# hccho2/Tacotron-Wavenet-Vocoder-Korean

Hardware: AMD Instinct MI355X
Metric: WaveNet autoregressive audio samples/sec at 24 kHz, batch=8 (higher is better)
Workload: dtype f32

## Files before the change

tacotron-wavenet-vocoder-korean_amd/csrc/twv_dpp.hpp:

```cpp
#pragma once
#include <hip/hip_runtime.h>
#include "twv_math.hpp"

#define TWV_ALIGN8 "\t.p2align 3\n"

namespace twv {

__host__ __device__ inline int dpp_a(int n) { return 4 * (n >> 1) + (n & 1); }
__host__ __device__ inline int dpp_conv_out(int lane) { const int r = lane >> 4, n = lane & 15; return ((r >> 1) ? 32 : 0) + dpp_a(n) + ((r & 1) ? 2 : 0); }
__host__ __device__ inline int dpp_dense_out(int lane) { return (lane & 15) + 16 * (lane >> 5); }
__host__ __device__ inline int dpp_dense_k(int lane, int i) { return dpp_a(i) + (((lane >> 4) & 1) ? 2 : 0); }
__host__ __device__ inline int dpp_z_index(int lane) { return dpp_a(lane & 15) + (((lane >> 4) & 1) ? 2 : 0); }

__device__ __forceinline__ float dot32_dpp(const float (&w)[32], float xa, float xb, float init = 0.0f)
{
    float c0 = init, c1 = 0.0f, c2 = 0.0f, c3 = 0.0f;
    asm volatile(
        "s_nop 1\n" TWV_ALIGN8
        "v_fmac_f32_dpp %0, %4, %5 row_newbcast:0 row_mask:0xf bank_mask:0xf\n"
        "v_fmac_f32_dpp %1, %4, %6 row_newbcast:1 row_mask:0xf bank_mask:0xf\n"
        "v_fmac_f32_dpp %2, %4, %7 row_newbcast:2 row_mask:0xf bank_mask:0xf\n"
        "v_fmac_f32_dpp %3, %4, %8 row_newbcast:3 row_mask:0xf bank_mask:0xf\n"
        "v_fmac_f32_dpp %0, %4, %9 row_newbcast:4 row_mask:0xf bank_mask:0xf\n"
        "v_fmac_f32_dpp %1, %4, %10 row_newbcast:5 row_mask:0xf bank_mask:0xf\n"
// ... 153 lines not shown
    TWV_FMAC12_DPP(c, d, e, xb0, xb1, xb2, wa, wb, wc, 24, 8, 9, 10, 11);
    TWV_FMAC12_DPP(c, d, e, xb0, xb1, xb2, wa, wb, wc, 28, 12, 13, 14, 15);
    ra = (c[0] + c[1]) + (c[2] + c[3]);
    rb = (d[0] + d[1]) + (d[2] + d[3]);
    rc = (e[0] + e[1]) + (e[2] + e[3]);
}

__device__ __forceinline__ float dot16_dpp(const float (&w)[16], float z, float init = 0.0f)
{
    float c0 = init, c1 = 0.0f;
    asm volatile(
        "s_nop 1\n" TWV_ALIGN8
        "v_fmac_f32_dpp %0, %2, %3 row_newbcast:0 row_mask:0xf bank_mask:0xf\n"
        "v_fmac_f32_dpp %1, %2, %4 row_newbcast:1 row_mask:0xf bank_mask:0xf\n"
        "v_fmac_f32_dpp %0, %2, %5 row_newbcast:2 row_mask:0xf bank_mask:0xf\n"
        "v_fmac_f32_dpp %1, %2, %6 row_newbcast:3 row_mask:0xf bank_mask:0xf\n"
        "v_fmac_f32_dpp %0, %2, %7 row_newbcast:4 row_mask:0xf bank_mask:0xf\n"
        "v_fmac_f32_dpp %1, %2, %8 row_newbcast:5 row_mask:0xf bank_mask:0xf\n"
        "v_fmac_f32_dpp %0, %2, %9 row_newbcast:6 row_mask:0xf bank_mask:0xf\n"
        "v_fmac_f32_dpp %1, %2, %10 row_newbcast:7 row_mask:0xf bank_mask:0xf\n"
        "v_fmac_f32_dpp %0, %2, %11 row_newbcast:8 row_mask:0xf bank_mask:0xf\n"
        "v_fmac_f32_dpp %1, %2, %12 row_newbcast:9 row_mask:0xf bank_mask:0xf\n"
        "v_fmac_f32_dpp %0, %2, %13 row_newbcast:10 row_mask:0xf bank_mask:0xf\n"
        "v_fmac_f32_dpp %1, %2, %14 row_newbcast:11 row_mask:0xf bank_mask:0xf\n"
        "v_fmac_f32_dpp %0, %2, %15 row_newbcast:12 row_mask:0xf bank_mask:0xf\n"
        "v_fmac_f32_dpp %1, %2, %16 row_newbcast:13 row_mask:0xf bank_mask:0xf\n"
        "v_fmac_f32_dpp %0, %2, %17 row_newbcast:14 row_mask:0xf bank_mask:0xf\n"
        "v_fmac_f32_dpp %1, %2, %18 row_newbcast:15 row_mask:0xf bank_mask:0xf"
        : "+v"(c0), "+v"(c1)
        : "v"(z), "v"(w[0]), "v"(w[1]), "v"(w[2]), "v"(w[3]), "v"(w[4]), "v"(w[5]), "v"(w[6]), "v"(w[7]), "v"(w[8]), "v"(w[9]), "v"(w[10]), "v"(w[11]), "v"(w[12]), "v"(w[13]), "v"(w[14]), "v"(w[15]));
    return c0 + c1;
}

__device__ __forceinline__ float dot32_dpp_chain(const float (&w)[32], float xa, float xb, float init)
{
    float c0 = init, c1, c2, c3;
    asm volatile(
        "s_nop 1\n" TWV_ALIGN8
        "v_fmac_f32_dpp %0, %4, %5 row_newbcast:0 row_mask:0xf bank_mask:0xf\n"
        "v_mul_f32_dpp %1, %4, %6 row_newbcast:1 row_mask:0xf bank_mask:0xf\n"
        "v_mul_f32_dpp %2, %4, %7 row_newbcast:2 row_mask:0xf bank_mask:0xf\n"
        "v_mul_f32_dpp %3, %4, %8 row_newbcast:3 row_mask:0xf bank_mask:0xf\n"
        "v_fmac_f32_dpp %0, %4, %9 row_newbcast:4 row_mask:0xf bank_mask:0xf\n"
        "v_fmac_f32_dpp %1, %4, %10 row_newbcast:5 row_mask:0xf bank_mask:0xf\n"
        "v_fmac_f32_dpp %2, %4, %11 row_newbcast:6 row_mask:0xf bank_mask:0xf\n"
        "v_fmac_f32_dpp %3, %4, %12 row_newbcast:7 row_mask:0xf bank_mask:0xf\n"
        "v_fmac_f32_dpp %0, %4, %13 row_newbcast:8 row_mask:0xf bank_mask:0xf\n"
        "v_fmac_f32_dpp %1, %4, %14 row_newbcast:9 row_mask:0xf bank_mask:0xf\n"
        "v_fmac_f32_dpp %2, %4, %15 row_newbcast:10 row_mask:0xf bank_mask:0xf\n"
        "v_fmac_f32_dpp %3, %4, %16 row_newbcast:11 row_mask:0xf bank_mask:0xf\n"
        "v_fmac_f32_dpp %0, %4, %17 row_newbcast:12 row_mask:0xf bank_mask:0xf\n"
        "v_fmac_f32_dpp %1, %4, %18 row_newbcast:13 row_mask:0xf bank_mask:0xf\n"
        "v_fmac_f32_dpp %2, %4, %19 row_newbcast:14 row_mask:0xf bank_mask:0xf\n"
        "v_fmac_f32_dpp %3, %4, %20 row_newbcast:15 row_mask:0xf bank_mask:0xf"
        : "+v"(c0), "=&v"(c1), "=&v"(c2), "=&v"(c3)
        : "v"(xa), "v"(w[0]), "v"(w[1]), "v"(w[2]), "v"(w[3]), "v"(w[4]), "v"(w[5]), "v"(w[6]), "v"(w[7]), "v"(w[8]), "v"(w[9]), "v"(w[10]), "v"(w[11]), "v"(w[12]), "v"(w[13]), "v"(w[14]), "v"(w[15]));
    asm volatile(
        TWV_ALIGN8
        "v_fmac_f32_dpp %0, %4, %5 row_newbcast:0 row_mask:0xf bank_mask:0xf\n"
        "v_fmac_f32_dpp %1, %4, %6 row_newbcast:1 row_mask:0xf bank_mask:0xf\n"
        "v_fmac_f32_dpp %2, %4, %7 row_newbcast:2 row_mask:0xf bank_mask:0xf\n"
        "v_fmac_f32_dpp %3, %4, %8 row_newbcast:3 row_mask:0xf bank_mask:0xf\n"
        "v_fmac_f32_dpp %0, %4, %9 row_newbcast:4 row_mask:0xf bank_mask:0xf\n"
        "v_fmac_f32_dpp %1, %4, %10 row_newbcast:5 row_mask:0xf bank_mask:0xf\n"
        "v_fmac_f32_dpp %2, %4, %11 row_newbcast:6 row_mask:0xf bank_mask:0xf\n"
        "v_fmac_f32_dpp %3, %4, %12 row_newbcast:7 row_mask:0xf bank_mask:0xf\n"
// ... 111 lines not shown
```

tacotron-wavenet-vocoder-korean_amd/csrc/twv_wavenet_xcd.hip:

```cpp
#include <hip/hip_runtime.h>
#include <stdint.h>
#include <string>
#include <type_traits>
#include "../../include/twv_amd.h"
#include "twv_layout.hpp"
#include "twv_math.hpp"
#include "twv_dev.hpp"
#include "twv_dpp.hpp"
#include "twv_categorical.hpp"
#include "twv_xcd.hpp"

using namespace twv;

#ifndef TWV_CHAIN_PAD
#define TWV_CHAIN_PAD 0
#endif
#ifndef TWV_WATCHDOG_LOG2
#define TWV_WATCHDOG_LOG2 21
#endif
#define TWV_STR2(x) #x
#define TWV_STR(x) TWV_STR2(x)
namespace {

typedef __attribute__((address_space(1))) unsigned long long gu64;
// ... 107 lines not shown
        "v_fmac_f32_dpp %1, %4, %6 row_newbcast:1 row_mask:0xf bank_mask:0xf\n"
        "v_fmac_f32_dpp %2, %4, %7 row_newbcast:2 row_mask:0xf bank_mask:0xf\n"
        "v_fmac_f32_dpp %3, %4, %8 row_newbcast:3 row_mask:0xf bank_mask:0xf\n"
        "v_fmac_f32_dpp %0, %4, %9 row_newbcast:4 row_mask:0xf bank_mask:0xf\n"
        "v_fmac_f32_dpp %1, %4, %10 row_newbcast:5 row_mask:0xf bank_mask:0xf\n"
        "v_fmac_f32_dpp %2, %4, %11 row_newbcast:6 row_mask:0xf bank_mask:0xf\n"
        "v_fmac_f32_dpp %3, %4, %12 row_newbcast:7 row_mask:0xf bank_mask:0xf\n"
        "v_fmac_f32_dpp %0, %4, %13 row_newbcast:8 row_mask:0xf bank_mask:0xf\n"
        "v_fmac_f32_dpp %1, %4, %14 row_newbcast:9 row_mask:0xf bank_mask:0xf\n"
        "v_fmac_f32_dpp %2, %4, %15 row_newbcast:10 row_mask:0xf bank_mask:0xf\n"
        "v_fmac_f32_dpp %3, %4, %16 row_newbcast:11 row_mask:0xf bank_mask:0xf\n"
        "v_fmac_f32_dpp %0, %4, %17 row_newbcast:12 row_mask:0xf bank_mask:0xf\n"
        "v_fmac_f32_dpp %1, %4, %18 row_newbcast:13 row_mask:0xf bank_mask:0xf\n"
        "v_fmac_f32_dpp %2, %4, %19 row_newbcast:14 row_mask:0xf bank_mask:0xf\n"
        "v_fmac_f32_dpp %3, %4, %20 row_newbcast:15 row_mask:0xf bank_mask:0xf"
        : "+v"(c0), "+v"(c1), "+v"(c2), "+v"(c3)
        : "v"(xb), "v"(w[0]), "v"(w[1]), "v"(w[2]), "v"(w[3]), "v"(w[4]), "v"(w[5]), "v"(w[6]), "v"(w[7]), "v"(w[8]), "v"(w[9]), "v"(w[10]), "v"(w[11]), "v"(w[12]), "v"(w[13]), "v"(w[14]), "v"(w[15]));
    return (c0 + c1) + (c2 + c3);
}

#define XSTAMP(cond_, slot_) do { if ((INSTR & 1) && a.prof != nullptr && b == a.prof_stream && t < a.prof_steps && lane == 0 && (cond_)) a.prof[(long long)t * 64 + (slot_)] = wall_clock64(); } while (0)

#define WACC_DECL() unsigned long long wacc_[6] = {0, 0, 0, 0, 0, 0}, w0_ = 0, wt0_ = 0; if (INSTR & 4) wt0_ = __builtin_amdgcn_s_memtime()
#define WACC_T0() do { if (INSTR & 4) w0_ = __builtin_amdgcn_s_memtime(); } while (0)
#define WACC_T1(i_) do { if (INSTR & 4) wacc_[i_] += __builtin_amdgcn_s_memtime() - w0_; } while (0)
constexpr int kTraceStep = 2000;
#define WTRACE(cond_, slot_) do { if ((INSTR & 4) && a.prof != nullptr && t == kTraceStep && (cond_) && lane == 0) a.prof[2048 + (slot_)] = wall_clock64(); } while (0)
#define WACC_OUT(prof_, slot_, wave_) do { if ((INSTR & 4) && (prof_) != nullptr && (slot_) >= 0 && lane == 0) {                 \
        unsigned long long* o_ = (prof_) + (((slot_) * 8 + (wave_)) * 8);                                                        \
        o_[0] = __builtin_amdgcn_s_memtime() - wt0_;                                                                             \
        o_[1] = wacc_[0]; o_[2] = wacc_[1]; o_[3] = wacc_[2]; o_[4] = wacc_[3]; o_[5] = wacc_[4]; o_[6] = wacc_[5]; } } while (0)
#define XMARK(role_, stage_) do { if ((INSTR & 1) && lane == 0) xb_store(rs, (int)XcdExch::MARK + (role_) * 8 + (int)(threadIdx.x >> 6), 0, (unsigned)t + 1u, (float)(stage_)); } while (0)

enum { ROLE_CHAIN = 0, ROLE_SERVICE = 1, ROLE_SKIP0 = 2, ROLE_CONV0 = 10, ROLE_LC0 = 18 };
constexpr int kXcdStreamsPerXcd = kXcdStreams / 8;

struct XArgs {
    XcdLaunch p;
    int n_lc_wg, lc_lpw;
    int total_roles;
};

template <int NS> struct XStreams { rsrc_t rs[NS]; int b[NS]; };
__device__ __forceinline__ rsrc_t exch_rsrc(const XcdLaunch& a, int b)
{
    return __builtin_amdgcn_make_buffer_rsrc(a.exch + (long long)b * XcdExch::WORDS, 0, (int)(XcdExch::WORDS * 8), 0x00020000);
}
struct XLazyRs { const XcdLaunch* a; int xcc, ns; __device__ __forceinline__ rsrc_t operator[](int k) const { return exch_rsrc(*a, xcc + 8 * (k < ns ? k : 0)); } };
struct XLazyB { int xcc, ns; __device__ __forceinline__ int operator[](int k) const { return xcc + 8 * (k < ns ? k : 0); } };
template <int NS> struct XStreamsLazy { XLazyRs rs; XLazyB b; };
constexpr int kSkipLdsWords = 32 * 64;
constexpr int kConvLdsFloats = 16 * 64 + 64;

constexpr int kChainLpw = 5;
template <int INSTR, bool ALL, bool FORCED, bool SEG1, bool TWOSEG, int NC, bool ONEHOT = false, bool HEAD = false, bool CONT = false>
__device__ __forceinline__ void chain_role(const XArgs& xa, int b, rsrc_t rs)
{
    const XcdLaunch& a = xa.p;
    const Layout& L = a.lay;
    const int w = __builtin_amdgcn_readfirstlane(threadIdx.x >> 6), lane = threadIdx.x & 63;
    const int NL = L.NL, T = a.T;
    const bool use_bias = L.use_bias != 0, has_gc = L.G > 0, has_lc = L.L > 0;
    constexpr bool forced = FORCED;
    constexpr int kLayerWaves = kXcdSeg0Layers / kChainLpw;
    const int l0 = (SEG1 ? kXcdSeg0Layers : 0) + kChainLpw * w;
    const int lw0 = kChainLpw * w;
    const int cap = (HEAD || w >= kLayerWaves) ? 0 : kChainLpw;
    int nl = NL - l0;
    nl = nl < 0 ? 0 : (nl > cap ? cap : nl);
    const int nlc = NC >= 0 ? NC : nl;
    const bool next_has = (l0 + nl < NL);
    constexpr bool head = HEAD;
// ... 677 lines not shown
            if (!havez) qz = xb_load_t<BAR>(rs, (int)XcdExch::ZX + last_layer * 128, zc_lane * 2);
            q = xb_load_t<BAR>(rs, (int)XcdExch::H1 + v * 64, lane);
            if (!havez && __all(g_tag(qz) == tag)) {
                const auto sw = __builtin_amdgcn_permlane32_swap((unsigned)qz, (unsigned)qz, false, false);
                val = dot32_dpp(wl, __uint_as_float(sw[0]), __uint_as_float(sw[1]));
                if (use_bias) val = val + bl;
                havez = true;
                saw_z = true;
            }
            if (havez && __all(g_tag(q) == tag)) break;
            if (!poll_tick<BAR>(pl, 61)) break;
            if (!havez) __builtin_amdgcn_s_sleep(1);
        }
        const float tot = g_val(q) + val;
        const float h = tot > 0.0f ? tot : 0.0f;
        q = (unsigned long long)__float_as_uint(h);
    } else {
        for (;;) {
            q = xb_load_t<BAR>(rs, (int)XcdExch::H1 + v * 64, lane);
            if (__all(g_tag(q) == tag)) break;
            if (!poll_tick<BAR>(pl, 61)) break;
            __builtin_amdgcn_s_sleep(1);
        }
    }
    return q;
}
__device__ __forceinline__ void conv1_load_last_skip(const XcdLaunch& a, const int v, const int lane, Tile& wl, float& bl)
{
    const Layout& L = a.lay;
    const long long lb = L.off_layer0 + (long long)(L.NL - 1) * L.layer_stride;
    load_tile(wl, a.P + lb + LayerOff::SK + (long long)v * kTile, lane);
    if (L.use_bias != 0) bl = a.P[lb + LayerOff::SK + (long long)L.NSJ * kTile + v * 64 + lane];
}

template <int INSTR, int NS, bool BAR = false, class SX = XStreams<NS>, int KF = 0>
__device__ __forceinline__ void conv1_role(const XArgs& xa, const SX& sx, int g, const int ns_rt = NS, const int prof_slot = -1)
{
    const XcdLaunch& a = xa.p;
    const Layout& L = a.lay;
    const int v = __builtin_amdgcn_readfirstlane(threadIdx.x >> 6), lane = threadIdx.x & 63;
    const int T = a.T, NCH = L.NCH;
    const bool use_bias = L.use_bias != 0;
    Poll pl{sx.rs[0], a.status, 0, false};
    constexpr int O_PART = 0, O_CNT = 16 * 64;
    if (threadIdx.x < NS) LDSI(threadIdx.x * kConvLdsFloats + O_CNT) = 0;
    __syncthreads();
    const int c0 = 2 * v, c1 = 2 * v + 1;
    Tile ta, tb;
    load_tile(ta, a.P + L.off_w1 + ((long long)g * NCH + c0) * kTile, lane);
    load_tile(tb, a.P + L.off_w1 + ((long long)g * NCH + c1) * kTile, lane);
    const bool summer = v < 2;
    float b1v = 0.0f;
    Tile t2;
    if (summer) {
        if (use_bias) b1v = a.P[L.off_b1 + g * 64 + lane];
        load_tile(t2, a.P + L.off_w2 + (long long)(2 * g + v) * kTile, lane);
    }
    Tile wl;
    float bl = 0.0f;
    if (KF > 0) conv1_load_last_skip(a, v, lane, wl, bl);
    const int zc_lane = lane_of_z((lane < 32 ? 0 : 16) + (lane & 15));
    unsigned long long t_arr = 0, period = 0;
    WACC_DECL();
    for (int t = 0; t < T && !pl.dead; ++t) {
        asm volatile(".p2align 6");
        const unsigned tag = (unsigned)t + 1u;
        WACC_T0();
        if (period) nap_until(t_arr + period - (period >> 3));
        WACC_T1(0);
#pragma unroll
        for (int k = 0; k < NS; ++k) {
            if (pl.dead) break;
            if (k >= ns_rt) break;
            const rsrc_t rs = sx.rs[k];
            const int b = sx.b[k];
            const int ob = k * kConvLdsFloats;
            pl.rs = rs;
            XMARK(ROLE_CONV0 + g, 1);
            WACC_T0();
            bool saw_z = false;
            const unsigned long long q = conv1_fetch_h1<KF, BAR>(pl, rs, v, lane, tag, L.NL - 1, zc_lane, wl.w, bl, use_bias, saw_z);
            (void)saw_z;
            WACC_T1(1);
            WTRACE(prof_slot >= 0 && k == 0, 400 + g * 8 + v);
            unsigned long long now_arr = 0;
            if (k == 0) now_arr = __builtin_amdgcn_s_memtime();
            XSTAMP(g == 0 && v == 0, 22);
            const unsigned hq = (unsigned)q;
            const auto p16 = __builtin_amdgcn_permlane16_swap(hq, hq, false, false);
            const auto pa = __builtin_amdgcn_permlane32_swap(p16[0], p16[0], false, false);
            const auto pb = __builtin_amdgcn_permlane32_swap(p16[1], p16[1], false, false);
            float r0, r1;
            dot32_dpp_x2(ta.w, __uint_as_float(pa[0]), __uint_as_float(pb[0]), tb.w, __uint_as_float(pa[1]), __uint_as_float(pb[1]), r0, r1);
            lds[ob + O_PART + c0 * 64 + lane] = r0;
            lds[ob + O_PART + c1 * 64 + lane] = r1;
            asm volatile("" ::: "memory");
            if (lane == 0) __hip_atomic_fetch_add(&LDSI(ob + O_CNT), 1, __ATOMIC_RELAXED, __HIP_MEMORY_SCOPE_WORKGROUP);
            if (k == 0) {
                const unsigned long long d = now_arr - t_arr;
                period = (t_arr != 0 && d < (1ull << 18)) ? d : 0;
                t_arr = now_arr;
            }
            XSTAMP(g == 0 && v == 0, 23);
            XMARK(ROLE_CONV0 + g, 2);
            if (summer) {
                WACC_T0();
                pl.it = 0;
                while (LDSVI(ob + O_CNT) < 8 * (t + 1)) { if (!poll_tick<BAR>(pl, 62)) break; }
                WACC_T1(2);
                asm volatile("" ::: "memory");
                XSTAMP(g == 0 && v == 0, 24);
                float cp[16];
#pragma unroll
                for (int ch = 0; ch < 16; ++ch) cp[ch] = lds[ob + O_PART + ch * 64 + lane];
                __builtin_amdgcn_sched_barrier(0);
                float r = cp[0];
#pragma unroll
                for (int ch = 1; ch < 16; ++ch) r = r + cp[ch];
                if (use_bias) r = r + b1v;
                const float h = r > 0.0f ? r : 0.0f;
                const float p = (v == 0) ? dot_readlane_pipe(t2, h) : dot_readlane_pipe32(t2, h);
                if (lane < 32) xb_store(rs, (int)XcdExch::PT, (g * 32 + lane) * 2 + v, tag, p);
                WTRACE(prof_slot >= 0 && k == 0, 480 + g * 2 + v);
                XSTAMP(g == 0 && v == 0, 25);
            }
        }
    }
    if (pl.dead && lane == 0) {
#pragma unroll
        for (int k = 0; k < NS; ++k) xb_store(sx.rs[k], (int)XcdExch::CTRL + 1, 0, 1u, 0.0f);
    }
    WACC_OUT(a.prof, prof_slot, v);
}

constexpr int kConvQLdsFloats = 16 * 64 + 64 + 8 * 64;
template <int INSTR, int NS, int KF = 0>
__device__ __forceinline__ void conv1_onehot_role(const XArgs& xa, const XStreams<NS>& sx, int g)
{
    const XcdLaunch& a = xa.p;
    const Layout& L = a.lay;
    const int v = __builtin_amdgcn_readfirstlane(threadIdx.x >> 6), lane = threadIdx.x & 63;
    const int T = a.T, NCH = L.NCH;
    const bool use_bias = L.use_bias != 0;
    Poll pl{sx.rs[0], a.status, 0, false};
    constexpr int O_PART = 0, O_CNT = 16 * 64, O_P2 = 16 * 64 + 64;
    if (threadIdx.x < NS) { LDSI(threadIdx.x * kConvQLdsFloats + O_CNT) = 0; LDSI(threadIdx.x * kConvQLdsFloats + O_CNT + 1) = 0; }
    __syncthreads();
    const int c0 = 2 * v, c1 = 2 * v + 1;
    Tile ta, tb;
    load_tile(ta, a.P + L.off_w1 + ((long long)g * NCH + c0) * kTile, lane);
    load_tile(tb, a.P + L.off_w1 + ((long long)g * NCH + c1) * kTile, lane);
    float w2[32];
    {
        const int ch2 = lane < 32 ? c0 : c1;
        const f32x4* src = reinterpret_cast<const f32x4*>(a.P + L.off_w2 + ((long long)(g >> 1) * NCH + ch2) * kTile) + ((g & 1) * 32 + (lane & 31));
#pragma unroll
        for (int q = 0; q < 8; ++q) { const f32x4 w = src[q * 64]; w2[4 * q] = w.x; w2[4 * q + 1] = w.y; w2[4 * q + 2] = w.z; w2[4 * q + 3] = w.w; }
    }
    float b1v = 0.0f, b2v = 0.0f;
    if (use_bias && v == 0) b1v = a.P[L.off_b1 + g * 64 + lane];
    if (use_bias && v == 1 && lane < 32) b2v = a.P[L.off_b2 + g * 32 + lane];
    Tile wl;
    float bl = 0.0f;
    if (KF > 0) conv1_load_last_skip(a, v, lane, wl, bl);
    const int zc_lane = lane_of_z((lane < 32 ? 0 : 16) + (lane & 15));
// ... 120 lines not shown
        }
    }
    const int o_row = v * 256;
    const int n16 = lane & 15;
    int ph[4] = {0, 0, 0, 0}, frame = 0;
    const int n_up = L.n_up;
    int hop = 1;
    for (int i = 0; i < n_up; ++i) hop *= L.up[i];
    const long long need_rows = (mode == XLC_MEL) ? ((long long)T + hop - 1) / hop : T;
    if (rows < need_rows) {
        if (lane == 0) {
            atomicMax(a.status, 71);
#pragma unroll
            for (int k = 0; k < NS; ++k) xb_store(sx.rs[k], (int)XcdExch::CTRL + 1, 0, 1u, 0.0f);
        }
        return;
    }
    WACC_DECL();
    for (int u = 0; u < T && !pl.dead; ++u) {
        const int t = u;
        float k0[4] = {0.f, 0.f, 0.f, 0.f}, k1[4] = {0.f, 0.f, 0.f, 0.f};
        if (mode != XLC_UPSAMPLED) {
#pragma unroll
            for (int i = 0; i < 4; ++i)
                if (i < n_up) { k0[i] = a.P[L.off_up[i] + ph[i] * 2 + 0]; k1[i] = a.P[L.off_up[i] + ph[i] * 2 + 1]; }
        }
        WACC_T0();
        if (u + 3 - kXcdLcRing > 0) {
#pragma unroll
            for (int k = 0; k < NS; ++k) {
                if (k >= ns_rt) break;
                const rsrc_t rs = sx.rs[k];
                pl.rs = rs;
                XMARK(ROLE_LC0 + wg, 1);
                pl.it = 0;
                while (!pl.dead) {
                    const unsigned long long q = xb_load_t<BAR>(rs, (int)XcdExch::CTRL, 0);
                    if ((int)g_tag(q) >= u + 3 - kXcdLcRing) break;
                    if (!poll_tick<BAR>(pl, 72)) break;
                    __builtin_amdgcn_s_sleep(16);
                }
            }
            if (pl.dead) break;
        }
        WACC_T1(0);
        float rowa[NS], rowb[NS];
#pragma unroll
        for (int k = 0; k < NS; ++k) {
            rowa[k] = 0.0f; rowb[k] = 0.0f;
            if (k >= ns_rt) continue;
            const float* src = payload + ((long long)sx.b[k] * rows + (mode == XLC_UPSAMPLED ? u : frame)) * Lc;
            rowa[k] = lane < Lc ? src[lane] : 0.0f;
            rowb[k] = 64 + lane < Lc ? src[64 + lane] : 0.0f;
        }
#pragma unroll
        for (int k = 0; k < NS; ++k) {
            if (k >= ns_rt) break;
            const rsrc_t rs = sx.rs[k];
            const int b = sx.b[k];
            int o_cur = o_row;
            lds[o_cur + lane] = rowa[k];
            lds[o_cur + 64 + lane] = rowb[k];
            if (mode != XLC_UPSAMPLED) {
#pragma unroll
                for (int i = 0; i < 4; ++i) {
                    if (i < n_up) {
                        const int o_nxt = (o_cur == o_row) ? o_row + 128 : o_row;
// ... 84 lines not shown
            f = atomicAdd(decision, 0);
            if (f != 0) break;
            __builtin_amdgcn_s_sleep(32);
        }
        if (f == 0) {
            const int old = atomicCAS(decision, 0, 2);
            f = old == 0 ? 2 : old;
            if (old == 0) atomicMax(a.status, 90);
        }
        s_go = (f == 1) ? 1 : 0;
    }
    __syncthreads();
    return s_go != 0;
}

template <int INSTR, bool BIGK, bool ONE, bool ONEHOT = false>
__global__ void __launch_bounds__(512) wn_xcd_generate_kernel(XArgs xa)
{
    const XcdLaunch& a = xa.p;
    unsigned xcc;
    asm volatile("s_getreg_b32 %0, hwreg(HW_REG_XCC_ID)" : "=s"(xcc));
    xcc &= 15u;
    int ticket = 0;
    if (threadIdx.x == 0) ticket = (xcc < (unsigned)a.B && xcc < 8u) ? atomicAdd(a.roles + xcc, 1) : 1 << 20;
    ticket = __shfl(ticket, 0);
    __shared__ int s_ticket;
    if (threadIdx.x == 0) s_ticket = ticket;
    for (int i = threadIdx.x; i < kXcdStreamsPerXcd * kSkipLdsWords * 2 + 64; i += blockDim.x) lds[i] = 0.0f;
    __syncthreads();
    ticket = s_ticket;
    const int ns = xcc < (unsigned)a.B && xcc < 8u ? (a.B - (int)xcc + 7) / 8 : 0;
    constexpr int nseg = BIGK ? 2 : 1;
    const int nchain = ns * nseg;
    if (ticket >= nchain + ns + 16 + xa.n_lc_wg) return;
    if (!roles_resident(xa)) return;
    const bool forced = a.forced != nullptr;
    auto exch_of = [&](int b) { return __builtin_amdgcn_make_buffer_rsrc(a.exch + (long long)b * XcdExch::WORDS, 0, (int)(XcdExch::WORDS * 8), 0x00020000); };
    if (ticket < nchain + ns) {
        const int k = ticket < nchain ? ticket / nseg : ticket - nchain;
        const int b = (int)xcc + 8 * k;
        const rsrc_t rs = exch_of(b);
        if (ticket < nchain) {
            if (ticket % nseg == 0) {
                const int wv = __builtin_amdgcn_readfirstlane(threadIdx.x >> 6);
                const int nlw = a.lay.NL - kChainLpw * wv;
                if (wv == 7) {
                    if (forced) chain_role<INSTR, true, true, false, BIGK, 0, ONEHOT, true>(xa, b, rs);
                    else chain_role<INSTR, true, false, false, BIGK, 0, ONEHOT, true>(xa, b, rs);
                }
                else if (wv >= kXcdSeg0Layers / kChainLpw || nlw <= 0) {}
                else if (forced) chain_role<INSTR, true, true, false, BIGK, -1, ONEHOT>(xa, b, rs);
                else if (nlw > kChainLpw) chain_role<INSTR, true, false, false, BIGK, kChainLpw, ONEHOT, false, true>(xa, b, rs);
                else if (nlw == kChainLpw) chain_role<INSTR, true, false, false, BIGK, kChainLpw, ONEHOT, false, false>(xa, b, rs);
                else chain_role<INSTR, true, false, false, BIGK, -1, ONEHOT>(xa, b, rs);
            } else if constexpr (BIGK) {
                const int wv = __builtin_amdgcn_readfirstlane(threadIdx.x >> 6);
                if (forced) chain_role<INSTR, true, true, true, true, -1>(xa, b, rs);
                else if (a.lay.NL - kXcdSeg0Layers - kChainLpw * wv >= kChainLpw) chain_role<INSTR, true, false, true, true, kChainLpw>(xa, b, rs);
                else chain_role<INSTR, true, false, true, true, -1>(xa, b, rs);
            }
        }
        else service_role<INSTR, BIGK>(xa, b, rs);
        return;
    }
    const int role = ticket - nchain - ns;
    auto shared_roles = [&](auto nsc) {
        constexpr int NS = decltype(nsc)::value;
        XStreams<NS> sx;
#pragma unroll
        for (int k = 0; k < NS; ++k) { sx.b[k] = (int)xcc + 8 * k; sx.rs[k] = exch_of(sx.b[k]); }
        constexpr int KF = TWV_XCD_KF;
        constexpr bool kUnfolded = KF == 0 || INSTR == 0;
        const bool fold = KF > 0 && (a.lay.NL > KF || !kUnfolded);
        if (role < 8) {
            if (!forced) {
                if (fold) skip_role<INSTR, NS, BIGK, KF>(xa, sx, role);
                else if constexpr (kUnfolded) skip_role<INSTR, NS, BIGK, 0>(xa, sx, role);
            }
        }
        else if (role < 16) {
            if (!forced) {
                if constexpr (ONEHOT) {
                    if (fold) conv1_onehot_role<INSTR, NS, KF>(xa, sx, role - 8);
                    else if constexpr (kUnfolded) conv1_onehot_role<INSTR, NS, 0>(xa, sx, role - 8);
                }
                else if (fold) conv1_role<INSTR, NS, false, XStreams<NS>, KF>(xa, sx, role - 8);
                else if constexpr (kUnfolded) conv1_role<INSTR, NS>(xa, sx, role - 8);
            }
        }
        else lc_role<INSTR, NS, BIGK>(xa, sx, role - 16);
    };
    if constexpr (BIGK) {
        if (ns == 1) shared_roles(std::integral_constant<int, 1>{});
        else shared_roles(std::integral_constant<int, 2>{});
    } else if constexpr (ONE) {
        shared_roles(std::integral_constant<int, 1>{});
    } else {
        if (ns == 1) shared_roles(std::integral_constant<int, 1>{});
        else if (ns == 2) shared_roles(std::integral_constant<int, 2>{});
        else if (ns == 3) shared_roles(std::integral_constant<int, 3>{});
        else shared_roles(std::integral_constant<int, 4>{});
    }
}

#define MMARK(rs_, slot_, stage_) do { if ((INSTR & 2) && lane == 0) xb_store(rs_, (int)XcdExch::MARK + (slot_), 0, (unsigned)t + 1u, (float)(stage_)); } while (0)
constexpr int kMS = 2;
constexpr int kManyChains = 6;
constexpr int kManyPerXcd = kMS * kManyChains;
constexpr int kM_BOX = 10;
constexpr int kM_OWD = 4096;
constexpr int kM_OGC = kM_OWD + kXcdSeg0Layers * 1024;
constexpr int kM_OHS = kM_OGC + kMS * kXcdSeg0Layers * 64;
constexpr int kManyChainLds = kM_OHS + kMS * 9 * 64;
constexpr int kManySkipData4 = kManyPerXcd * 8 * 64;
constexpr int kManySkipLds = kManySkipData4 * 4 + kManyPerXcd * 8 * 64;
constexpr int kManyLds = kManyChainLds > kManySkipLds ? kManyChainLds : kManySkipLds;


template <int INSTR>
__device__ __forceinline__ float many_sample(const XcdLaunch& a, const Layout& L, Poll& pl, rsrc_t rs, int lane, unsigned tag, float b2v,
                                             float s_lnl, float s_tq, bool use_bias, int b, int NL)
{
    const int half = lane >> 5;
// ... 825 lines not shown
                if (c == 0) v = blob[lb + (oc < 32 ? L.c_bf : L.c_bg) + (oc & 31)];
                else if (c == 1) v = blob[lb + L.c_bd + od];
            }
            dst[L.off_xl + i] = v;
        } else {
            const int e = (int)(i - per_layer * L.NL);
            const int q = e >> 8, lane = (e >> 2) & 63, c = e & 3;
            const int k = 4 * q + c;
            if (k < L.ifw) v = blob[L.c_causal + k * 32 + dpp_dense_out(lane)];
            dst[L.off_xc + e] = v;
        }
    }
}

}

namespace twv {

bool xcd_model_ok(const Layout& L)
{
    const bool head_ok = L.scalar ? (L.ifw == 32 && L.O <= 32 && L.NOJ == 1) : (L.Q == 256 && L.O == 256);
    return head_ok && L.S == 512 && L.NL >= 1 && L.NL <= kXcdMaxLayers && L.NLC <= 4;
}
static bool xcd_many_lc_fits(const Layout& L) { return (long long)kManyPerXcd * (L.n_up + 1) * L.NLC * 32 <= kManyLds / 8; }
int xcd_max_streams(const Layout& L) { return L.NL > kXcdSeg0Layers ? kXcdStreams / 2 : (L.scalar && xcd_many_lc_fits(L) ? kXcdManyStreams : kXcdStreams); }
static int lc_layers_per_wave(const Layout& L) { const int n = L.NLC > 0 ? (L.NL > kXcdSeg0Layers ? 6 : 4) / L.NLC : 1; return n < 1 ? 1 : (n > 4 ? 4 : n); }
int xcd_lc_workgroups(const Layout& L)
{
    if (L.L == 0) return 0;
    const int lpw = lc_layers_per_wave(L);
    const int waves = (L.NL + lpw - 1) / lpw;
    return (waves + 7) / 8;
}
int xcd_workgroups_per_stream(const Layout& L) { return ROLE_LC0 + xcd_lc_workgroups(L); }
size_t xcd_exchange_bytes(int batch) { return (size_t)batch * XcdExch::WORDS * 8 + 64; }
void xcd_pack(float* packed, const float* blob, const Layout& L, hipStream_t st)
{
    hipLaunchKernelGGL(wn_xcd_pack_kernel, dim3(512), dim3(256), 0, st, packed, blob, L);
}
bool xcd_uses_many(const Layout& L, int batch, int many_opt)
{
    return L.scalar && (batch > kXcdStreams || many_opt == 1 || (many_opt == 0 && batch >= kXcdManyFrom)) && L.NL <= kXcdSeg0Layers && xcd_many_lc_fits(L);
}
int xcd_launch(const XcdLaunch& p, hipStream_t st)
{
    XArgs xa;
    xa.p = p;
    xa.n_lc_wg = xcd_lc_workgroups(p.lay);
    xa.lc_lpw = lc_layers_per_wave(p.lay);
    const bool many = xcd_uses_many(p.lay, p.B, p.many);
    xa.total_roles = 0;
    for (int x = 0; x < 8 && x < p.B; ++x) {
        const int ns = (p.B - x + 7) / 8;
        if (many) xa.total_roles += 2 * ((ns + kMS - 1) / kMS) + 16 + xa.n_lc_wg;
        else xa.total_roles += ns * (p.lay.NL > kXcdSeg0Layers ? 2 : 1) + ns + 16 + xa.n_lc_wg;
    }
    const size_t shm = many ? (size_t)kManyLds * 4 : p.lay.NL > kXcdSeg0Layers ? (size_t)159 * 1024 : (size_t)kXcdChainLdsFloats * 4;
    int dev = 0, cus = 256;
    hipDeviceProp_t prop;
    if (hipGetDevice(&dev) == hipSuccess && hipGetDeviceProperties(&prop, dev) == hipSuccess) cus = prop.multiProcessorCount;
    else (void)hipGetLastError();
    const int grid = 2 * cus;
    const int instr = (p.prof != nullptr ? 1 : 0) | (p.dbg != nullptr ? 2 : 0);
    auto go = [&](auto kern) {
        (void)hipFuncSetAttribute((const void*)kern, hipFuncAttributeMaxDynamicSharedMemorySize, (int)shm);
        (void)hipGetLastError();
        hipLaunchKernelGGL(kern, dim3(grid), dim3(512), shm, st, xa);
    };
    if (!many && instr != 0 && p.lay.NL <= TWV_XCD_KF)
        return twv_fail(TWV_E_UNSUPPORTED, "layer dumps / phase stamps of the XCD kernel need a model of at least two layers (set option \"xcd\" = 0 for the generic kernel)");
    if (many) {
        if (p.B > kXcdManyStreams) return twv_fail(TWV_E_UNSUPPORTED, "the many-streams XCD kernel takes at most 96 streams");
        if (instr == 3) return twv_fail(TWV_E_UNSUPPORTED, "layer dumps and wait accounting are separate builds of the many-streams kernel");
        if (instr == 1) go(wn_xcd_many_kernel<4>);
        else if (instr == 2) go(wn_xcd_many_kernel<2>);
        else go(wn_xcd_many_kernel<0>);
    }
    else if (!p.lay.scalar) {
        if (p.B > (p.lay.NL > kXcdSeg0Layers ? kXcdStreams / 2 : kXcdStreams)) return twv_fail(TWV_E_UNSUPPORTED, "the one-hot XCD kernel takes at most 32 streams (16 above 30 layers)");
        if (instr == 3 || (instr != 0 && p.lay.NL > kXcdSeg0Layers))
            return twv_fail(TWV_E_UNSUPPORTED, "the one-hot XCD kernel has layer dumps OR phase stamps, up to 30 layers (set option \"xcd\" = 0 for the generic kernel)");
        if (p.lay.NL > kXcdSeg0Layers) go(wn_xcd_generate_kernel<0, true, false, true>);
        else if (instr == 2) go(wn_xcd_generate_kernel<2, false, false, true>);
        else if (instr == 1) go(wn_xcd_generate_kernel<1, false, false, true>);
        else if (p.B <= 8) go(wn_xcd_generate_kernel<0, false, true, true>);
        else go(wn_xcd_generate_kernel<0, false, false, true>);
    }
    else if (p.lay.NL > kXcdSeg0Layers) {
// ... 15 lines not shown
```

Baseline: 974,900.

## Split conv1 output-head role into two half-channel workgroups per group

Adds a conv1_half_role that splits each conv1 group's 64 output channels across two workgroups, so each wave does 16-wide DPP dot products instead of 32-wide, with permlane swaps for the reductions. The second 1x1 (w2) also moves to a half-tile DPP dot with a permlane16 reduction instead of readlane pipelines. The change raises the conv1 workgroup count from 8 to 16 per stream for batch<=8 scalar models and renumbers the LC roles to follow. The aim is to shorten the per-step critical path of the output head, at the cost of more resident workgroups and extra cross-workgroup coordination.

Measured after the change: 996,600 (median of 6 runs). 1.02x the previous value.

```diff
diff --git a/tacotron-wavenet-vocoder-korean_amd/csrc/twv_dpp.hpp b/tacotron-wavenet-vocoder-korean_amd/csrc/twv_dpp.hpp
--- a/tacotron-wavenet-vocoder-korean_amd/csrc/twv_dpp.hpp
+++ b/tacotron-wavenet-vocoder-korean_amd/csrc/twv_dpp.hpp
@@ -209,6 +209,53 @@
     return c0 + c1;
 }
 
+__device__ __forceinline__ void dot16_dpp_x2(const float (&wa)[16], float za, const float (&wb)[16], float zb, float& ra, float& rb)
+{
+    float c0 = 0.0f, c1 = 0.0f, d0 = 0.0f, d1 = 0.0f;
+    asm volatile(
+        "s_nop 1\n" TWV_ALIGN8
+        "v_fmac_f32_dpp %0, %4, %6 row_newbcast:0 row_mask:0xf bank_mask:0xf\n"
+        "v_fmac_f32_dpp %2, %5, %14 row_newbcast:0 row_mask:0xf bank_mask:0xf\n"
+        "v_fmac_f32_dpp %1, %4, %7 row_newbcast:1 row_mask:0xf bank_mask:0xf\n"
+        "v_fmac_f32_dpp %3, %5, %15 row_newbcast:1 row_mask:0xf bank_mask:0xf\n"
+        "v_fmac_f32_dpp %0, %4, %8 row_newbcast:2 row_mask:0xf bank_mask:0xf\n"
+        "v_fmac_f32_dpp %2, %5, %16 row_newbcast:2 row_mask:0xf bank_mask:0xf\n"
+        "v_fmac_f32_dpp %1, %4, %9 row_newbcast:3 row_mask:0xf bank_mask:0xf\n"
+        "v_fmac_f32_dpp %3, %5, %17 row_newbcast:3 row_mask:0xf bank_mask:0xf\n"
+        "v_fmac_f32_dpp %0, %4, %10 row_newbcast:4 row_mask:0xf bank_mask:0xf\n"
+        "v_fmac_f32_dpp %2, %5, %18 row_newbcast:4 row_mask:0xf bank_mask:0xf\n"
+        "v_fmac_f32_dpp %1, %4, %11 row_newbcast:5 row_mask:0xf bank_mask:0xf\n"
+        "v_fmac_f32_dpp %3, %5, %19 row_newbcast:5 row_mask:0xf bank_mask:0xf\n"
+        "v_fmac_f32_dpp %0, %4, %12 row_newbcast:6 row_mask:0xf bank_mask:0xf\n"
+        "v_fmac_f32_dpp %2, %5, %20 row_newbcast:6 row_mask:0xf bank_mask:0xf\n"
+        "v_fmac_f32_dpp %1, %4, %13 row_newbcast:7 row_mask:0xf bank_mask:0xf\n"
+        "v_fmac_f32_dpp %3, %5, %21 row_newbcast:7 row_mask:0xf bank_mask:0xf"
+        : "+v"(c0), "+v"(c1), "+v"(d0), "+v"(d1)
+        : "v"(za), "v"(zb), "v"(wa[0]), "v"(wa[1]), "v"(wa[2]), "v"(wa[3]), "v"(wa[4]), "v"(wa[5]), "v"(wa[6]), "v"(wa[7]), "v"(wb[0]), "v"(wb[1]), "v"(wb[2]), "v"(wb[3]), "v"(wb[4]), "v"(wb[5]), "v"(wb[6]), "v"(wb[7]));
+    asm volatile(
+        "s_nop 1\n" TWV_ALIGN8
+        "v_fmac_f32_dpp %0, %4, %6 row_newbcast:8 row_mask:0xf bank_mask:0xf\n"
+        "v_fmac_f32_dpp %2, %5, %14 row_newbcast:8 row_mask:0xf bank_mask:0xf\n"
+        "v_fmac_f32_dpp %1, %4, %7 row_newbcast:9 row_mask:0xf bank_mask:0xf\n"
+        "v_fmac_f32_dpp %3, %5, %15 row_newbcast:9 row_mask:0xf bank_mask:0xf\n"
+        "v_fmac_f32_dpp %0, %4, %8 row_newbcast:10 row_mask:0xf bank_mask:0xf\n"
+        "v_fmac_f32_dpp %2, %5, %16 row_newbcast:10 row_mask:0xf bank_mask:0xf\n"
+        "v_fmac_f32_dpp %1, %4, %9 row_newbcast:11 row_mask:0xf bank_mask:0xf\n"
+        "v_fmac_f32_dpp %3, %5, %17 row_newbcast:11 row_mask:0xf bank_mask:0xf\n"
+        "v_fmac_f32_dpp %0, %4, %10 row_newbcast:12 row_mask:0xf bank_mask:0xf\n"
+        "v_fmac_f32_dpp %2, %5, %18 row_newbcast:12 row_mask:0xf bank_mask:0xf\n"
+        "v_fmac_f32_dpp %1, %4, %11 row_newbcast:13 row_mask:0xf bank_mask:0xf\n"
+        "v_fmac_f32_dpp %3, %5, %19 row_newbcast:13 row_mask:0xf bank_mask:0xf\n"
+        "v_fmac_f32_dpp %0, %4, %12 row_newbcast:14 row_mask:0xf bank_mask:0xf\n"
+        "v_fmac_f32_dpp %2, %5, %20 row_newbcast:14 row_mask:0xf bank_mask:0xf\n"
+        "v_fmac_f32_dpp %1, %4, %13 row_newbcast:15 row_mask:0xf bank_mask:0xf\n"
+        "v_fmac_f32_dpp %3, %5, %21 row_newbcast:15 row_mask:0xf bank_mask:0xf"
+        : "+v"(c0), "+v"(c1), "+v"(d0), "+v"(d1)
+        : "v"(za), "v"(zb), "v"(wa[8]), "v"(wa[9]), "v"(wa[10]), "v"(wa[11]), "v"(wa[12]), "v"(wa[13]), "v"(wa[14]), "v"(wa[15]), "v"(wb[8]), "v"(wb[9]), "v"(wb[10]), "v"(wb[11]), "v"(wb[12]), "v"(wb[13]), "v"(wb[14]), "v"(wb[15]));
+    ra = c0 + c1;
+    rb = d0 + d1;
+}
+
 __device__ __forceinline__ float dot32_dpp_chain(const float (&w)[32], float xa, float xb, float init)
 {
     float c0 = init, c1, c2, c3;
diff --git a/tacotron-wavenet-vocoder-korean_amd/csrc/twv_wavenet_xcd.hip b/tacotron-wavenet-vocoder-korean_amd/csrc/twv_wavenet_xcd.hip
--- a/tacotron-wavenet-vocoder-korean_amd/csrc/twv_wavenet_xcd.hip
+++ b/tacotron-wavenet-vocoder-korean_amd/csrc/twv_wavenet_xcd.hip
@@ -163,12 +163,13 @@
         o_[1] = wacc_[0]; o_[2] = wacc_[1]; o_[3] = wacc_[2]; o_[4] = wacc_[3]; o_[5] = wacc_[4]; o_[6] = wacc_[5]; } } while (0)
 #define XMARK(role_, stage_) do { if ((INSTR & 1) && lane == 0) xb_store(rs, (int)XcdExch::MARK + (role_) * 8 + (int)(threadIdx.x >> 6), 0, (unsigned)t + 1u, (float)(stage_)); } while (0)
 
-enum { ROLE_CHAIN = 0, ROLE_SERVICE = 1, ROLE_SKIP0 = 2, ROLE_CONV0 = 10, ROLE_LC0 = 18 };
+enum { ROLE_CHAIN = 0, ROLE_SERVICE = 1, ROLE_SKIP0 = 2, ROLE_CONV0 = 10 };
 constexpr int kXcdStreamsPerXcd = kXcdStreams / 8;
 
 struct XArgs {
     XcdLaunch p;
     int n_lc_wg, lc_lpw;
+    int n_conv1;
     int total_roles;
 };
 
@@ -912,6 +913,21 @@
     load_tile(wl, a.P + lb + LayerOff::SK + (long long)v * kTile, lane);
     if (L.use_bias != 0) bl = a.P[lb + LayerOff::SK + (long long)L.NSJ * kTile + v * 64 + lane];
 }
+__device__ __forceinline__ void load_half_tile(float (&w)[16], const float* base, const int obase, const int lane)
+{
+    const float2* p = reinterpret_cast<const float2*>(base + (obase + dpp_dense_out(lane)) * 4 + (((lane >> 4) & 1) ? 2 : 0));
+#pragma unroll
+    for (int j = 0; j < 8; ++j) {
+        const float2 q = p[j * 128];
+        w[2 * j] = q.x; w[2 * j + 1] = q.y;
+    }
+}
+__device__ __forceinline__ float conv1d2_chunk_dpp(const float (&t2)[16], const float h)
+{
+    const float s = dot16_dpp(t2, h);
+    const auto ds = __builtin_amdgcn_permlane16_swap(__float_as_uint(s), __float_as_uint(s), false, false);
+    return __uint_as_float(ds[0]) + __uint_as_float(ds[1]);
+}
 
 template <int INSTR, int NS, bool BAR = false, class SX = XStreams<NS>, int KF = 0>
 __device__ __forceinline__ void conv1_role(const XArgs& xa, const SX& sx, int g, const int ns_rt = NS, const int prof_slot = -1)
@@ -930,11 +946,12 @@
     load_tile(ta, a.P + L.off_w1 + ((long long)g * NCH + c0) * kTile, lane);
     load_tile(tb, a.P + L.off_w1 + ((long long)g * NCH + c1) * kTile, lane);
     const bool summer = v < 2;
+    const int hz = 32 * v + dpp_z_index(lane);
     float b1v = 0.0f;
-    Tile t2;
+    float t2[16];
     if (summer) {
-        if (use_bias) b1v = a.P[L.off_b1 + g * 64 + lane];
-        load_tile(t2, a.P + L.off_w2 + (long long)(2 * g + v) * kTile, lane);
+        if (use_bias) b1v = a.P[L.off_b1 + g * 64 + hz];
+        load_half_tile(t2, a.P + L.off_w2 + (long long)(2 * g + v) * kTile, 0, lane);
     }
     Tile wl;
     float bl = 0.0f;
@@ -992,15 +1009,15 @@
                 XSTAMP(g == 0 && v == 0, 24);
                 float cp[16];
 #pragma unroll
-                for (int ch = 0; ch < 16; ++ch) cp[ch] = lds[ob + O_PART + ch * 64 + lane];
+                for (int ch = 0; ch < 16; ++ch) cp[ch] = lds[ob + O_PART + ch * 64 + hz];
                 __builtin_amdgcn_sched_barrier(0);
                 float r = cp[0];
 #pragma unroll
                 for (int ch = 1; ch < 16; ++ch) r = r + cp[ch];
                 if (use_bias) r = r + b1v;
                 const float h = r > 0.0f ? r : 0.0f;
-                const float p = (v == 0) ? dot_readlane_pipe(t2, h) : dot_readlane_pipe32(t2, h);
-                if (lane < 32) xb_store(rs, (int)XcdExch::PT, (g * 32 + lane) * 2 + v, tag, p);
+                const float p = conv1d2_chunk_dpp(t2, h);
+                if ((lane & 16) == 0) xb_store(rs, (int)XcdExch::PT, (g * 32 + dpp_dense_out(lane)) * 2 + v, tag, p);
                 WTRACE(prof_slot >= 0 && k == 0, 480 + g * 2 + v);
                 XSTAMP(g == 0 && v == 0, 25);
             }
@@ -1011,6 +1028,92 @@
         for (int k = 0; k < NS; ++k) xb_store(sx.rs[k], (int)XcdExch::CTRL + 1, 0, 1u, 0.0f);
     }
     WACC_OUT(a.prof, prof_slot, v);
+}
+
+template <int INSTR, int KF>
+__device__ __forceinline__ void conv1_half_role(const XArgs& xa, const XStreams<1>& sx, const int g, const int hh)
+{
+    static_assert(KF > 0, "the last layer's skip 1x1 runs here");
+    const XcdLaunch& a = xa.p;
+    const Layout& L = a.lay;
+    const int v = __builtin_amdgcn_readfirstlane(threadIdx.x >> 6), lane = threadIdx.x & 63;
+    const int T = a.T, NCH = L.NCH;
+    const bool use_bias = L.use_bias != 0;
+    const rsrc_t rs = sx.rs[0];
+    const int b = sx.b[0];
+    Poll pl{rs, a.status, 0, false};
+    constexpr int O_PART = 0, O_CNT = 16 * 64;
+    if (threadIdx.x == 0) LDSI(O_CNT) = 0;
+    __syncthreads();
+    const int c0 = 2 * v, c1 = 2 * v + 1;
+    float ta[16], tb[16];
+    load_half_tile(ta, a.P + L.off_w1 + ((long long)g * NCH + c0) * kTile, 32 * hh, lane);
+    load_half_tile(tb, a.P + L.off_w1 + ((long long)g * NCH + c1) * kTile, 32 * hh, lane);
+    const int zi = dpp_z_index(lane), od = dpp_dense_out(lane);
+    const int hl = 32 * (lane >> 5) + zi;
+    const bool summer = v == 0;
+    float b1v = 0.0f;
+    float t2[16];
+    if (summer) {
+        if (use_bias) b1v = a.P[L.off_b1 + g * 64 + 32 * hh + zi];
+        load_half_tile(t2, a.P + L.off_w2 + (long long)(2 * g + hh) * kTile, 0, lane);
+    }
+    Tile wl;
+    float bl = 0.0f;
+    conv1_load_last_skip(a, v, hl, wl, bl);
+    const int zc_lane = lane_of_z((lane < 32 ? 0 : 16) + (lane & 15));
+    unsigned long long t_arr = 0, period = 0;
+    for (int t = 0; t < T && !pl.dead; ++t) {
+        asm volatile(".p2align 6");
+        const unsigned tag = (unsigned)t + 1u;
+        if (period) nap_until(t_arr + period - (period >> 3));
+        XMARK(ROLE_CONV0 + 2 * g + hh, 1);
+        bool saw_z = false;
+        const unsigned long long q = conv1_fetch_h1<KF, false>(pl, rs, v, hl, tag, L.NL - 1, zc_lane, wl.w, bl, use_bias, saw_z);
+        (void)saw_z;
+        const unsigned long long now_arr = __builtin_amdgcn_s_memtime();
+        XSTAMP(g == 0 && hh == 0 && v == 0, 22);
+        const unsigned hq = (unsigned)q;
+        const auto hs = __builtin_amdgcn_permlane32_swap(hq, hq, false, false);
+        float s0, s1;
+        dot16_dpp_x2(ta, __uint_as_float(hs[0]), tb, __uint_as_float(hs[1]), s0, s1);
+        const auto d0 = __builtin_amdgcn_permlane16_swap(__float_as_uint(s0), __float_as_uint(s0), false, false);
+        const auto d1 = __builtin_amdgcn_permlane16_swap(__float_as_uint(s1), __float_as_uint(s1), false, false);
+        const float r0 = __uint_as_float(d0[0]) + __uint_as_float(d0[1]);
+        const float r1 = __uint_as_float(d1[0]) + __uint_as_float(d1[1]);
+        if ((lane & 16) == 0) {
+            lds[O_PART + c0 * 32 + od] = r0;
+            lds[O_PART + c1 * 32 + od] = r1;
+        }
+        asm volatile("" ::: "memory");
+        if (lane == 0) __hip_atomic_fetch_add(&LDSI(O_CNT), 1, __ATOMIC_RELAXED, __HIP_MEMORY_SCOPE_WORKGROUP);
+        {
+            const unsigned long long d = now_arr - t_arr;
+            period = (t_arr != 0 && d < (1ull << 18)) ? d : 0;
+            t_arr = now_arr;
+        }
+        XSTAMP(g == 0 && hh == 0 && v == 0, 23);
+        XMARK(ROLE_CONV0 + 2 * g + hh, 2);
+        if (summer) {
+            pl.it = 0;
+            while (LDSVI(O_CNT) < 8 * (t + 1)) { if (!poll_tick(pl, 62)) break; }
+            asm volatile("" ::: "memory");
+            XSTAMP(g == 0 && hh == 0, 24);
+            float cp[16];
+#pragma unroll
+            for (int ch = 0; ch < 16; ++ch) cp[ch] = lds[O_PART + ch * 32 + zi];
+            __builtin_amdgcn_sched_barrier(0);
+            float r = cp[0];
+#pragma unroll
+            for (int ch = 1; ch < 16; ++ch) r = r + cp[ch];
+            if (use_bias) r = r + b1v;
+            const float h = r > 0.0f ? r : 0.0f;
+            const float p = conv1d2_chunk_dpp(t2, h);
+            if ((lane & 16) == 0) xb_store(rs, (int)XcdExch::PT, (g * 32 + od) * 2 + hh, tag, p);
+            XSTAMP(g == 0 && hh == 0, 25);
+        }
+    }
+    if (pl.dead && lane == 0) xb_store(rs, (int)XcdExch::CTRL + 1, 0, 1u, 0.0f);
 }
 
 constexpr int kConvQLdsFloats = 16 * 64 + 64 + 8 * 64;
@@ -1197,7 +1300,7 @@
                 if (k >= ns_rt) break;
                 const rsrc_t rs = sx.rs[k];
                 pl.rs = rs;
-                XMARK(ROLE_LC0 + wg, 1);
+                XMARK(ROLE_CONV0 + xa.n_conv1 + wg, 1);
                 pl.it = 0;
                 while (!pl.dead) {
                     const unsigned long long q = xb_load_t<BAR>(rs, (int)XcdExch::CTRL, 0);
@@ -1348,7 +1451,8 @@
     const int ns = xcc < (unsigned)a.B && xcc < 8u ? (a.B - (int)xcc + 7) / 8 : 0;
     constexpr int nseg = BIGK ? 2 : 1;
     const int nchain = ns * nseg;
-    if (ticket >= nchain + ns + 16 + xa.n_lc_wg) return;
+    const int nc1 = xa.n_conv1;
+    if (ticket >= nchain + ns + 8 + nc1 + xa.n_lc_wg) return;
     if (!roles_resident(xa)) return;
     const bool forced = a.forced != nullptr;
     auto exch_of = [&](int b) { return __builtin_amdgcn_make_buffer_rsrc(a.exch + (long long)b * XcdExch::WORDS, 0, (int)(XcdExch::WORDS * 8), 0x00020000); };
@@ -1394,8 +1498,12 @@
                 else if constexpr (kUnfolded) skip_role<INSTR, NS, BIGK, 0>(xa, sx, role);
             }
         }
-        else if (role < 16) {
+        else if (role < 8 + nc1) {
             if (!forced) {
+                constexpr bool kHalf = !ONEHOT && !BIGK && NS == 1 && KF > 0 && (ONE || INSTR != 0);
+                if constexpr (kHalf) {
+                    if (nc1 == 16) { conv1_half_role<INSTR, KF>(xa, sx, (role - 8) >> 1, (role - 8) & 1); return; }
+                }
                 if constexpr (ONEHOT) {
                     if (fold) conv1_onehot_role<INSTR, NS, KF>(xa, sx, role - 8);
                     else if constexpr (kUnfolded) conv1_onehot_role<INSTR, NS, 0>(xa, sx, role - 8);
@@ -1404,7 +1512,7 @@
                 else if constexpr (kUnfolded) conv1_role<INSTR, NS>(xa, sx, role - 8);
             }
         }
-        else lc_role<INSTR, NS, BIGK>(xa, sx, role - 16);
+        else lc_role<INSTR, NS, BIGK>(xa, sx, role - 8 - nc1);
     };
     if constexpr (BIGK) {
         if (ns == 1) shared_roles(std::integral_constant<int, 1>{});
@@ -2296,7 +2404,7 @@
     const int waves = (L.NL + lpw - 1) / lpw;
     return (waves + 7) / 8;
 }
-int xcd_workgroups_per_stream(const Layout& L) { return ROLE_LC0 + xcd_lc_workgroups(L); }
+int xcd_workgroups_per_stream(const Layout& L) { return ROLE_CONV0 + 8 + xcd_lc_workgroups(L); }
 size_t xcd_exchange_bytes(int batch) { return (size_t)batch * XcdExch::WORDS * 8 + 64; }
 void xcd_pack(float* packed, const float* blob, const Layout& L, hipStream_t st)
 {
@@ -2313,11 +2421,12 @@
     xa.n_lc_wg = xcd_lc_workgroups(p.lay);
     xa.lc_lpw = lc_layers_per_wave(p.lay);
     const bool many = xcd_uses_many(p.lay, p.B, p.many);
+    xa.n_conv1 = (!many && p.B <= 8 && p.lay.scalar && p.lay.NL <= kXcdSeg0Layers && p.lay.NL > TWV_XCD_KF && TWV_XCD_KF > 0) ? 16 : 8;
     xa.total_roles = 0;
     for (int x = 0; x < 8 && x < p.B; ++x) {
         const int ns = (p.B - x + 7) / 8;
-        if (many) xa.total_roles += 2 * ((ns + kMS - 1) / kMS) + 16 + xa.n_lc_wg;
-        else xa.total_roles += ns * (p.lay.NL > kXcdSeg0Layers ? 2 : 1) + ns + 16 + xa.n_lc_wg;
+        if (many) xa.total_roles += 2 * ((ns + kMS - 1) / kMS) + 8 + xa.n_conv1 + xa.n_lc_wg;
+        else xa.total_roles += ns * (p.lay.NL > kXcdSeg0Layers ? 2 : 1) + ns + 8 + xa.n_conv1 + xa.n_lc_wg;
     }
     const size_t shm = many ? (size_t)kManyLds * 4 : p.lay.NL > kXcdSeg0Layers ? (size_t)159 * 1024 : (size_t)kXcdChainLdsFloats * 4;
     int dev = 0, cus = 256;
```
